# kcoost/fast_speech_enhancement_metrics

Measured on AMD Instinct MI355X. Metric: utterances/sec PESQ-wb+STOI, 10s@16kHz, batch 4096, 1/2/4/8 MI355X, higher is better.
Workload: dtype f32; 1 GPU; PESQ-wb + STOI/ESTOI of 10 s @ 16 kHz fp32 pairs through the drop-in call PESQ_STOI(16000, use_gpu=True)(c, n) (fused joint entry, one read of the inputs) -> list of dicts; batch_per_gpu=4096, global_batch=4096, length=160000, parallelism=dp1 (utterance shards, RCCL all-gather of scores)

## Files before the change

### fast_speech_enhancement_metrics_amd/csrc/fsem_stoi.h

```cpp
#pragma once
#include "fsem_fft.h"
#include "fsem_resample.h"
#include "fsem_vad.h"

namespace fsem {
namespace stoi {

constexpr int NB = 15;
constexpr int NSEG = 30;
constexpr int VF = 64;
#ifndef FSEM_TOB_TF
#define FSEM_TOB_TF 32
#endif
constexpr int TF = FSEM_TOB_TF;
constexpr float kClip = 1.0f + 5.62341325190349f;

struct Rows {
  const int32_t *lens;
  int64_t ncap;
  int orig, nw;
  __device__ __forceinline__ int64_t n(int64_t b) const {
    if (!lens) return ncap;
    const int64_t v = lens[b];
    return v < 0 ? 0 : (v > ncap ? ncap : v);
  }
  __device__ __forceinline__ int64_t l10(int64_t b) const { return (n(b) * nw + orig - 1) / orig; }
  __device__ __forceinline__ int nv(int64_t b) const {
    const int64_t L10 = l10(b);
    return L10 >= 256 ? (int)((L10 - 256) / 128 + 1) : 0;
  }
};

__device__ __forceinline__ uint32_t peak_exponents(float c0, float c1, float c2, float c3, float d0, float d1,
                                                   float d2, float d3) {
  typedef unsigned short us2 __attribute__((ext_vector_type(2)));
  auto mx4 = [](float a, float b, float c, float d) {
    return __float_as_uint(__builtin_fmaxf(__builtin_fmaxf(__builtin_fabsf(a), __builtin_fabsf(b)),
                                           __builtin_fmaxf(__builtin_fabsf(c), __builtin_fabsf(d))));
  };
  const uint32_t mc = mx4(c0, c1, c2, c3), md = mx4(d0, d1, d2, d3);
  uint32_t e = ((mc >> 7) & 0xffff0000u) | (md >> 23);
  auto pmax = [](uint32_t x, uint32_t y) {
    return __builtin_bit_cast(uint32_t, __builtin_elementwise_max(__builtin_bit_cast(us2, x), __builtin_bit_cast(us2, y)));
  };
  e = pmax(e, dpp_mov<0x121>(e));
  e = pmax(e, dpp_mov<0x122>(e));
  e = pmax(e, dpp_mov<0x124>(e));
  e = pmax(e, dpp_mov<0x128>(e));
  e = pmax(e, (uint32_t)__builtin_amdgcn_update_dpp(0, (int)e, 0x142, 0xA, 0xF, false));
  e = pmax(e, (uint32_t)__builtin_amdgcn_update_dpp(0, (int)e, 0x143, 0xC, 0xF, false));
  return __builtin_amdgcn_readlane(e, 63);
}

#ifndef FSEM_SEG_T
#define FSEM_SEG_T 256
#endif
constexpr int SEG_T = FSEM_SEG_T;

inline int seg_blocks(int64_t tmax) { return tmax > 29 ? (int)((tmax - 29 + SEG_T - 1) / SEG_T) : 1; }

struct Geometry {
  int64_t L10;
  int NV, nv_ld, tmax;
  int64_t v_ld;
  int64_t y_ld;
  bool direct;
  int mode;
};

inline int make_geometry(int64_t length, int32_t sr, Geometry *g, ResampleKernel *rk) {
  g->direct = (sr == 10000);
  if (g->direct) {
    g->L10 = length;
    rk->orig = rk->nw = 1;
    rk->taps = 1;
    rk->width = 0;
  } else {
    const int rc = make_resample_kernel(sr, 10000, rk);
    if (rc != FSEM_OK) return rc;
    g->L10 = (rk->nw * length + rk->orig - 1) / rk->orig;
  }
  g->NV = g->L10 >= 256 ? (int)((g->L10 - 256) / 128 + 1) : 0;
  g->nv_ld = (int)align_up((size_t)(g->NV > 0 ? g->NV : 1), 64);
  g->v_ld = vad_ld(g->L10);
  g->tmax = g->NV > 2 ? g->NV - 2 : 1;
  g->y_ld = (int64_t)align_up((size_t)g->L10, 64);
  g->mode = g->direct ? 1 : ((sr == 16000) ? 0 : 2);
  return FSEM_OK;
}

struct Ws {
  float2 *vad;
  int *idx, *kept;
  float *tob;
  double *part;
  float *y10;
};
inline Ws layout(Arena &a, int64_t B, const Geometry &g) {
  Ws w;
  w.vad = a.take<float2>((size_t)B * (size_t)g.v_ld);
  w.idx = a.take<int>((size_t)B * g.nv_ld);
  w.kept = a.take<int>((size_t)B);
  w.tob = a.take<float>((size_t)(2 * B) * NB * (size_t)g.tmax);
  w.part = a.take<double>(2 * (size_t)B * (size_t)seg_blocks(g.tmax));
  w.y10 = a.take<float>((size_t)(2 * B) * (size_t)g.y_ld);
  return w;
}

int run(const float *ref, const float *deg, int64_t B, int64_t length, int64_t ld, const int32_t *lengths,
        int32_t sr, float *stoi_out, float *estoi_out, int32_t *kept_out, float *tob_out, int64_t tob_ld, void *ws,
        size_t ws_size, hipStream_t st);

}
}
```

### fast_speech_enhancement_metrics_amd/csrc/stoi.hip

```cpp
#include <algorithm>

#include "fsem_internal.h"
#include "fsem_stoi.h"

namespace fsem {
namespace stoi {

struct Src {
  const float *x;
  int64_t n;
};

__device__ __forceinline__ float sample10(const Src &s, int64_t o, int64_t L10, bool direct,
                                          const ResampleKernel &rk) {
  if (o < 0 || o >= L10) return 0.f;
  return direct ? s.x[o] : resample_at(s.x, s.n, o, rk);
}

__device__ __forceinline__ void vad_chunk(const float *__restrict__ y, int n, float2 *__restrict__ vrow, int tid,
                                          float4 wa, float4 wb) {
  const int lane = tid & 63, grp = tid >> 4;
  const float4 *__restrict__ y4 = reinterpret_cast<const float4 *>(y);
  for (int j0 = 0; 64 * j0 < n; j0 += 16) {
    const int j = j0 + grp;
    const bool full = 64 * j + 64 <= n;
    const float4 v = full ? y4[16 * j + (lane & 15)] : make_float4(0.f, 0.f, 0.f, 0.f);
    const float e = vad_quarter(v, wa, wb, lane);
    if ((lane & 14) == 0 && full) reinterpret_cast<float *>(vrow)[2 * j + (lane & 1)] = e;
  }
}

constexpr int VF2 = 32;
constexpr int YT = VF2 * 128 + 128;
constexpr int NG = YT / 5 + 2;
constexpr int XT4 = (8 * NG + 32) / 4;
constexpr int XPF = (XT4 + 255) / 256;
__global__ void __launch_bounds__(256, 2)
    stoi_resample_vad16(const float *__restrict__ ref, const float *__restrict__ deg, Rows rows, int64_t ld,
                        int nchunk, int64_t nitems, float *__restrict__ y10, int64_t y_ld,
                        float2 *__restrict__ vad, int64_t v_ld) {
  __shared__ __attribute__((aligned(16))) float xin[XPF * 256 * 4 + 4];
  __shared__ __attribute__((aligned(16))) float ytile[YT + 8];
  const int tid = threadIdx.x, lane = tid & 63;
  const int wave = __builtin_amdgcn_readfirstlane(tid >> 6);
  auto item_src = [&](int64_t item, int64_t &b, int &chunk, int &sig, int64_t &o0, int64_t &i0) {
    sig = (int)(item & 1);
    const int64_t bc = item >> 1;
    b = bc / nchunk;
    chunk = (int)(bc - b * nchunk);
    o0 = (int64_t)chunk * (VF2 * 128);
    i0 = 8 * (o0 / 5) - 12;
  };
  auto prefetch = [&](int64_t item, float4 pre[XPF]) {
    int64_t b, o0, i0;
    int chunk, sig;
    item_src(item, b, chunk, sig, o0, i0);
    const int64_t n_in = rows.n(b);
    const uint32_t nbytes = (uint32_t)(((n_in + 3) & ~(int64_t)3) * 4);
    const float *row = (sig == 0 ? ref : deg) + b * ld;
    const uint64_t base = reinterpret_cast<uint64_t>(row);
    const uint32_t lo = __builtin_amdgcn_readfirstlane((uint32_t)base);
    const uint32_t hi = __builtin_amdgcn_readfirstlane((uint32_t)(base >> 32));
    void *p = reinterpret_cast<void *>(((uint64_t)hi << 32) | lo);
    const __amdgpu_buffer_rsrc_t rsrc =
        __builtin_amdgcn_make_buffer_rsrc(p, 0, __builtin_amdgcn_readfirstlane(nbytes), 0x00020000);
#pragma unroll
    for (int k = 0; k < XPF; ++k) {
      const int64_t t = i0 + 4 * (tid + 256 * k);
      typedef float v4f __attribute__((ext_vector_type(4)));
      v4f v = __builtin_bit_cast(v4f, __builtin_amdgcn_raw_buffer_load_b128(rsrc, (int)(t * 4), 0, 0));
      if (t + 3 >= n_in) {
        v.x = (t < n_in) ? v.x : 0.f;
        v.y = (t + 1 < n_in) ? v.y : 0.f;
        v.z = (t + 2 < n_in) ? v.z : 0.f;
        v.w = 0.f;
      }
      pre[k] = make_float4(v.x, v.y, v.z, v.w);
    }
  };
  float4 vwa, vwb;
  vad_windows(lane, (tid >> 4) & 1, vwa, vwb);
  float4 pre[XPF];
  int64_t item = blockIdx.x;
  if (item < nitems) prefetch(item, pre);
  for (; item < nitems; item += gridDim.x) {
    int64_t b, o0, i0;
    int chunk, sig;
    item_src(item, b, chunk, sig, o0, i0);
    const int64_t L10 = rows.l10(b);
    if (o0 >= L10) {
      if (item + gridDim.x < nitems) prefetch(item + gridDim.x, pre);
      continue;
    }
    float2 *x2 = reinterpret_cast<float2 *>(xin + 2);
#pragma unroll
    for (int k = 0; k < XPF; ++k) {
      x2[2 * (tid + 256 * k)] = make_float2(pre[k].x, pre[k].y);
      x2[2 * (tid + 256 * k) + 1] = make_float2(pre[k].z, pre[k].w);
    }
    lds_barrier();
    if (item + gridDim.x < nitems) prefetch(item + gridDim.x, pre);
    const int64_t o_end = min(o0 + (int64_t)YT, L10);
    const int64_t m0 = o0 / 5;
    const int64_t m1 = (o_end + 4) / 5;
    for (int64_t m = m0 + tid; m < m1; m += 256) {
      const float4 *xs4 = reinterpret_cast<const float4 *>(xin + 8 * (m - m0) + 4);
      float v[28];
#pragma unroll
      for (int t = 0; t < 7; ++t) {
        const float4 q = xs4[t];
        v[4 * t] = q.x;
        v[4 * t + 1] = q.y;
        v[4 * t + 2] = q.z;
        v[4 * t + 3] = q.w;
      }
#pragma unroll
      for (int j = 0; j < 5; ++j) {
        float acc = 0.f;
#pragma unroll
        for (int t = 0; t < 28; ++t) acc = fmaf(kRs16k10k[j][t], v[t], acc);
        const int64_t o = 5 * m + j;
        if (o >= o0 && o < o_end) ytile[o - o0] = acc;
      }
    }
    lds_barrier();
    const int nown = (int)min((int64_t)(VF2 * 128), L10 - o0);
    float *__restrict__ yr = y10 + (b * 2 + sig) * y_ld + o0;
    for (int k = tid; 4 * k < nown; k += 256) {
      if (4 * k + 3 < nown) {
        reinterpret_cast<float4 *>(yr)[k] = reinterpret_cast<const float4 *>(ytile)[k];
      } else {
        for (int c = 4 * k; c < nown; ++c) yr[c] = ytile[c];
      }
    }
    if (sig == 0) vad_chunk(ytile, nown, vad + b * v_ld + (o0 >> 6), tid, vwa, vwb);
    lds_barrier();
  }
}

constexpr int VF3 = 32;
constexpr int YT3 = VF3 * 128 + 128;
__global__ void __launch_bounds__(256)
    stoi_resample_vad(const float *__restrict__ ref, const float *__restrict__ deg, Rows rows, int64_t ld,
                      int mode, ResampleKernel rk, float *__restrict__ y10, int64_t y_ld,
                      float2 *__restrict__ vad, int64_t v_ld, int64_t b0) {
  __shared__ __attribute__((aligned(16))) float ytile[YT3];
  const int tid = threadIdx.x, lane = tid & 63;
  const int64_t b = b0 + blockIdx.y;
  const int64_t o0 = (int64_t)blockIdx.x * (VF3 * 128);
  const int64_t n_in = rows.n(b), L10 = rows.l10(b);
  if (o0 >= L10) return;
  const int64_t o_end = min(o0 + (int64_t)YT3, L10);
  const int ny = (int)(o_end - o0);
  const int nw_own = (int)min((int64_t)(VF3 * 128), L10 - o0);
  float4 vwa, vwb;
  vad_windows(lane, (tid >> 4) & 1, vwa, vwb);
  for (int sig = 0; sig < 2; ++sig) {
    const Src src{(sig == 0 ? ref : deg) + b * ld, n_in};
    for (int k = tid; k < ny; k += 256) ytile[k] = sample10(src, o0 + k, L10, mode == 1, rk);
    lds_barrier();
    float *__restrict__ yr = y10 + (b * 2 + sig) * y_ld + o0;
    for (int k = tid; k < nw_own; k += 256) yr[k] = ytile[k];
    if (sig == 0) vad_chunk(ytile, nw_own, vad + b * v_ld + (o0 >> 6), tid, vwa, vwb);
    lds_barrier();
  }
}

constexpr int VQ = 4096;
__global__ void __launch_bounds__(256)
    stoi_vad10(const float *__restrict__ y10, int64_t y_ld, Rows rows, float2 *__restrict__ vad, int64_t v_ld,
               int64_t b0) {
  const int64_t b = b0 + blockIdx.y;
  const int64_t o0 = (int64_t)blockIdx.x * VQ;
  const int64_t L10 = rows.l10(b);
  if (o0 >= L10) return;
  float4 vwa, vwb;
  vad_windows(threadIdx.x & 63, (threadIdx.x >> 4) & 1, vwa, vwb);
  vad_chunk(y10 + (2 * b) * y_ld + o0, (int)min((int64_t)VQ, L10 - o0), vad + b * v_ld + (o0 >> 6), threadIdx.x, vwa,
            vwb);
}

__global__ void __launch_bounds__(256)
    stoi_select(const float2 *__restrict__ vad, int64_t v_ld, int nv_ld, Rows rows, int *__restrict__ idx,
                int *__restrict__ kept) {
  __shared__ float red[8];
  __shared__ int wcount[4];
  const int tid = threadIdx.x, lane = tid & 63;
  const int wave = __builtin_amdgcn_readfirstlane(tid >> 6);
  const int64_t b = blockIdx.x;
  const int NV = rows.nv(b);
  const float2 *__restrict__ q = vad + b * v_ld;
  float m = -INFINITY;
  int nan_seen = 0;
  for (int i = tid; i < NV; i += 256) {
    const float e = vad_energy_db(q, i);
    m = fmaxf(m, e);
    nan_seen |= (e != e);
  }
  m = block_max_256(m, red);
  const float thr = __syncthreads_or(nan_seen) ? __builtin_nanf("") : m - 40.f;
  int base = 0;
  for (int i0 = 0; i0 < NV; i0 += 256) {
    const int i = i0 + tid;
    const bool keep = (i < NV) && ((thr - vad_energy_db(q, i)) < 0.f);
    const unsigned long long bal = __ballot(keep);
    const int pre = __popcll(bal & ((1ull << lane) - 1ull));
    if (lane == 0) wcount[wave] = __popcll(bal);
    lds_barrier();
    int off = base;
    for (int w = 0; w < wave; ++w) off += wcount[w];
    if (keep) idx[b * nv_ld + off + pre] = i;
    base += wcount[0] + wcount[1] + wcount[2] + wcount[3];
    lds_barrier();
  }
  if (tid == 0) kept[b] = base;
}

#ifdef FSEM_STAMPS
constexpr int kTobStampBlocks = 131072;
__device__ unsigned long long g_tob_stamps[kTobStampBlocks][4];
#define TSTAMP(i)                                                                            \
  do {                                                                                       \
    const unsigned lin_ = blockIdx.y * gridDim.x + blockIdx.x;                               \
    if (threadIdx.x == 0 && lin_ < kTobStampBlocks) g_tob_stamps[lin_][i] = __builtin_amdgcn_s_memtime(); \
  } while (0)
#else
#define TSTAMP(i) \
  do {            \
  } while (0)
#endif

constexpr int TOB_PB = 264;
__device__ __forceinline__ constexpr int tob_pw(int k) { return k + (k >= 128 ? 3 : 0); }
constexpr bool tob_pieces_unsplit() {
  for (int l = 0; l < 64; ++l)
    if (kObmPiece[l][2] < 128 && kObmPiece[l][3] > 128) return false;
  return true;
}
static_assert(tob_pieces_unsplit() && 2 * TOB_PB <= 2 * kFftBuf - 12, "padded band-sum layout");

constexpr int TOB_WAVES = 4;
__global__ void __launch_bounds__(64 * TOB_WAVES)
    stoi_tob(const float *__restrict__ y10, int64_t y_ld, int64_t B, Rows rows, const int *__restrict__ idx,
             const int *__restrict__ kept, int nv_ld, float *__restrict__ tob, int64_t tmax, int64_t b0) {
  __shared__ __attribute__((aligned(16))) float blk[2][TF + 1][128];
  __shared__ __attribute__((aligned(16))) float xbuf[TOB_WAVES * 2 * kFftBuf];
  const int tid = threadIdx.x, lane = tid & 63;
  const int wave = __builtin_amdgcn_readfirstlane(tid >> 6);
  const int64_t b = b0 + blockIdx.y;
  const int n = kept[b];
  const int T = n - 2;
  const int64_t L10 = rows.l10(b);
  const int k0 = blockIdx.x * TF;
  if (k0 >= T) return;
  TSTAMP(0);
  const int kend = min(k0 + TF, T);
  const int *kidx = idx + b * nv_ld;
  const float *__restrict__ yc = y10 + (b * 2) * y_ld;
  const float *__restrict__ yd = yc + y_ld;
  auto row_rsrc = [L10](const float *y) {
    const uint64_t base = reinterpret_cast<uint64_t>(y);
    const uint32_t lo = __builtin_amdgcn_readfirstlane((uint32_t)base);
    const uint32_t hi = __builtin_amdgcn_readfirstlane((uint32_t)(base >> 32));
    void *p = reinterpret_cast<void *>(((uint64_t)hi << 32) | lo);
    return __builtin_amdgcn_make_buffer_rsrc(p, 0, __builtin_amdgcn_readfirstlane((uint32_t)(L10 * 4)), 0x00020000);
  };
  const __amdgpu_buffer_rsrc_t rc = row_rsrc(yc), rd = row_rsrc(yd);
  auto at = [](__amdgpu_buffer_rsrc_t r, int64_t o) {
    return __builtin_bit_cast(float, __builtin_amdgcn_raw_buffer_load_b32(r, (int)(o * 4), 0, 0));
  };
  const float w_lo = kHann256s[lane], w_lo2 = kHann256s[lane + 64];
  const float w_hi = kHann256s[128 + lane], w_hi2 = kHann256s[128 + 64 + lane];

  const int nblk = kend - k0 + 1;
  constexpr int NBW = (TF + 1 + TOB_WAVES - 1) / TOB_WAVES;
  float g[NBW][8];
#pragma unroll
  for (int u = 0; u < NBW; ++u) {
    const int j = min(wave + TOB_WAVES * u, nblk - 1);
    const int q = k0 + 1 + j;
    const int iq = kidx[q], ip = kidx[q - 1];
    const int64_t a0 = 128LL * iq, a1 = 128LL * ip + 128;
    g[u][0] = at(rc, a0 + lane);
    g[u][1] = at(rc, a1 + lane);
    g[u][2] = at(rc, a0 + 64 + lane);
    g[u][3] = at(rc, a1 + 64 + lane);
    g[u][4] = at(rd, a0 + lane);
    g[u][5] = at(rd, a1 + lane);
    g[u][6] = at(rd, a0 + 64 + lane);
    g[u][7] = at(rd, a1 + 64 + lane);
  }
#pragma unroll
  for (int u = 0; u < NBW; ++u) {
    const int j = wave + TOB_WAVES * u;
    if (j < nblk) {
      blk[0][j][lane] = w_lo * g[u][0] + w_hi * g[u][1];
      blk[0][j][64 + lane] = w_lo2 * g[u][2] + w_hi2 * g[u][3];
      blk[1][j][lane] = w_lo * g[u][4] + w_hi * g[u][5];
      blk[1][j][64 + lane] = w_lo2 * g[u][6] + w_hi2 * g[u][7];
    }
  }
  lds_stores_done();
  lds_barrier();
  TSTAMP(1);

  cf tw1[8], tw2[8];
  fft512_twiddles(lane, tw1, tw2);
  const float win[4] = {w_lo, w_lo2, w_hi, w_hi2};
  float2 *wbuf = reinterpret_cast<float2 *>(xbuf) + wave * kFftBuf;
  float *pbuf = reinterpret_cast<float *>(wbuf);
  const int plane = (64 - lane) & 63;
  const int pc_sig = kObmPiece[lane][0], pc_band = kObmPiece[lane][1];
  const int pc_lo = kObmPiece[lane][2], pc_hi = kObmPiece[lane][3];
  const int pc_at = TOB_PB * pc_sig + tob_pw(pc_lo);
  const int pc_gs = kObmPiece[lane][4];
  const bool pc_head = kObmPiece[lane][5] != 0;
  const int nfr = kend - k0;
  const int nfft = 2 * ((nfr + 1) >> 1);
  for (int f = wave; f < nfft; f += TOB_WAVES) {
    const int sg = f & 1;
    const int ja = 2 * (f >> 1);
    const bool has_b = ja + 1 < nfr;
    cf v[8];
#pragma unroll
    for (int r = 0; r < 4; ++r) {
      const int t = lane + 64 * (r & 1);
      const float a = blk[sg][ja + (r >> 1)][t];
      const float bq = has_b ? blk[sg][ja + 1 + (r >> 1)][t] : 0.f;
      v[r] = {a * win[r], bq * win[r]};
    }
#pragma unroll
    for (int r = 4; r < 8; ++r) v[r] = {0.f, 0.f};
    const uint32_t pk = peak_exponents(v[0].r, v[1].r, v[2].r, v[3].r, v[0].i, v[1].i, v[2].i, v[3].i);
    const int ea = (int)(pk >> 16), eb = (int)(pk & 0xffffu);
    const bool a_zero = ea == 0 && !__any(v[0].r != 0.f || v[1].r != 0.f || v[2].r != 0.f || v[3].r != 0.f);
    const bool b_zero = eb == 0 && !__any(v[0].i != 0.f || v[1].i != 0.f || v[2].i != 0.f || v[3].i != 0.f);
    int sh = (ea > 0 && eb > 0) ? ea - eb : 0;
    sh = (sh >= 7 || sh <= -7) ? max(-60, min(60, sh)) : 0;
    if (sh != 0) {
#pragma unroll
      for (int r = 0; r < 4; ++r) v[r].i = __builtin_amdgcn_ldexpf(v[r].i, sh);
    }
    const float a_scale = a_zero ? 0.f : 0.5f;
    const float b_scale = b_zero ? 0.f : __builtin_amdgcn_ldexpf(0.5f, -sh);
    fft512_wave<true>(v, wbuf, lane, tw1, tw2);
    float pa[4], pb[4];
#pragma unroll
    for (int r = 0; r < 4; ++r) {
      float mr = __shfl(v[7 - r].r, plane, 64);
      float mi = __shfl(v[7 - r].i, plane, 64);
      if (lane == 0) {
        mr = v[(8 - r) & 7].r;
        mi = v[(8 - r) & 7].i;
      }
      typedef float f2v __attribute__((ext_vector_type(2)));
      const f2v z = {v[r].r, v[r].i}, m = {mr, mi};
      const f2v sm = z + m;
      const f2v df = z.yx - m.yx;
      const f2v pp = __builtin_elementwise_fma(sm, sm, df * df);
      pa[r] = pp.x;
      pb[r] = pp.y;
    }
#pragma unroll
    for (int r = 0; r < 4; ++r) {
      pbuf[tob_pw(64 * r) + lane] = pa[r];
      pbuf[TOB_PB + tob_pw(64 * r) + lane] = pb[r];
    }
    wave_lds_fence();
    {
      const float *ps = pbuf + pc_at;
      float acc = (pc_lo < pc_hi) ? ps[0] : 0.f;
#pragma unroll
      for (int i = 1; i < 12; ++i) {
        const float x = ps[i];
        acc += (pc_lo + i < pc_hi) ? x : 0.f;
      }
      {
        const float a1 = __builtin_bit_cast(float, __builtin_amdgcn_update_dpp(0, __builtin_bit_cast(int, acc), 0x101, 0xF, 0xF, true));
        acc += (pc_gs >= 2) ? a1 : 0.f;
        const float a2 = __builtin_bit_cast(float, __builtin_amdgcn_update_dpp(0, __builtin_bit_cast(int, acc), 0x102, 0xF, 0xF, true));
        acc += (pc_gs >= 4) ? a2 : 0.f;
      }
      if (pc_head && (pc_sig == 0 || has_b))
        tob[((b + sg * B) * NB + pc_band) * tmax + k0 + ja + pc_sig] =
            __builtin_amdgcn_sqrtf(acc) * (pc_sig ? b_scale : a_scale);
    }
    wave_lds_fence();
  }
  TSTAMP(2);
}

#ifndef FSEM_SEG_OCC
#define FSEM_SEG_OCC 3
#endif
constexpr int SEG_WAVES = SEG_T / 64;
typedef float f2 __attribute__((ext_vector_type(2)));
__global__ void __launch_bounds__(SEG_T, FSEM_SEG_OCC)
    stoi_seg(const float *__restrict__ tob, int64_t B, int64_t tmax, const int *__restrict__ kept,
             double *__restrict__ part, int P, int64_t b0) {
  constexpr int W = SEG_T + NSEG;
  constexpr int LDX = W + 1;
  __shared__ f2 XY[NB][LDX];
  __shared__ double red[2 * SEG_WAVES];
  const int tid = threadIdx.x;
  const int64_t b = b0 + blockIdx.y;
  const int p = blockIdx.x;
  const int n = kept[b];
  const int S = n - 31;
  const int m0 = p * SEG_T;
  if (m0 >= S) return;
  const int T = n - 2;
  const float *xc = tob + (b * NB) * tmax;
  const float *xd = tob + ((b + B) * NB) * tmax;
  double st = 0.0, et = 0.0;
  constexpr float kInvN = 1.f / NSEG;
  {
    const int nf = min(W, T - m0);
    {
      f2 va[NB], vb[NB];
      const int t2 = tid + SEG_T;
      const int ia = min(tid, nf - 1), ib = min(t2, nf - 1);
#pragma unroll
      for (int j = 0; j < NB; ++j) {
        const float *xr = xc + j * tmax + m0, *dr = xd + j * tmax + m0;
        va[j] = (f2){xr[ia], dr[ia]};
        vb[j] = (f2){xr[ib], dr[ib]};
      }
#pragma unroll
      for (int j = 0; j < NB; ++j) {
        XY[j][tid] = va[j];
        if (t2 < W) XY[j][t2] = vb[j];
      }
    }
    lds_barrier();
    const int m = m0 + tid;
    if (m < S) {
      float s_acc = 0.f;
      f2 rxy[NB], nmr[NB];
      f2 nvar = {0.f, 0.f};
#pragma unroll 1
      for (int j = 0; j < NB; ++j) {
        f2 v[NSEG];
        f2 s1 = {0.f, 0.f};
#pragma unroll
        for (int t = 0; t < NSEG; ++t) {
          v[t] = XY[j][tid + t];
          s1 += v[t];
        }
        const f2 mu = s1 * kInvN;
        f2 dd = {0.f, 0.f};
#pragma unroll
        for (int t = 0; t < NSEG; ++t) {
          v[t] = v[t] - mu;
          dd = __builtin_elementwise_fma(v[t], v[t], dd);
        }
        const f2 s2 = __builtin_elementwise_fma(mu * (float)NSEG, mu, dd);
        const float alpha = __builtin_amdgcn_sqrtf(s2.x) * __builtin_amdgcn_rcpf(__builtin_amdgcn_sqrtf(s2.y) + 1e-9f);
        const f2 sc = {kClip, alpha};
        const f2 smu = sc * mu;
        static_assert(NSEG % 2 == 0, "frame pairs");
        f2 c[NSEG / 2];
        f2 syc2 = {0.f, 0.f};
#pragma unroll
        for (int u = 0; u < NSEG / 2; ++u) {
          const f2 q0 = __builtin_elementwise_fma(v[2 * u], sc, smu), q1 = __builtin_elementwise_fma(v[2 * u + 1], sc, smu);
          c[u] = (f2){fminf(q0.y, q0.x), fminf(q1.y, q1.x)};
          syc2 += c[u];
        }
        const float myc = (syc2.x + syc2.y) * kInvN;
        const f2 myc2 = {myc, myc};
        f2 dcc2 = {0.f, 0.f};
        float dxc = 0.f;
#pragma unroll
        for (int u = 0; u < NSEG / 2; ++u) {
          const f2 dc = c[u] - myc2;
          dcc2 = __builtin_elementwise_fma(dc, dc, dcc2);
          dxc = fmaf(v[2 * u].x, dc.x, dxc);
          dxc = fmaf(v[2 * u + 1].x, dc.y, dxc);
        }
        const float dcc = dcc2.x + dcc2.y;
        constexpr float kReg30 = 30e-24f;
        const float rxn = __builtin_amdgcn_rsqf(dd.x + kReg30);
        const float ryn = __builtin_amdgcn_rsqf(dd.y + kReg30);
        const float rcn = __builtin_amdgcn_rsqf(dcc + kReg30);
        s_acc = fmaf(dxc * rxn, rcn, s_acc) + (__builtin_isfinite(alpha) ? 0.f : __builtin_nanf(""));
        rxy[j] = (f2){rxn, ryn};
        nvar = __builtin_elementwise_fma(rxy[j], rxy[j], nvar);
        nmr[j] = -mu * rxy[j];
      }
      const f2 breg = __builtin_elementwise_fma(nvar, (f2){14e-24f / 15.f, 14e-24f / 15.f}, (f2){15e-24f, 15e-24f});
      float e_acc = 0.f;
      for (int t = 0; t < NSEG; ++t) {
        f2 a[NB];
        f2 ma = {0.f, 0.f};
#pragma unroll
        for (int j = 0; j < NB; ++j) {
          a[j] = __builtin_elementwise_fma(XY[j][tid + t], rxy[j], nmr[j]);
          ma += a[j];
        }
        ma *= 1.f / NB;
        f2 q = {0.f, 0.f};
        float ac = 0.f;
#pragma unroll
        for (int j = 0; j < NB; ++j) {
          const f2 d = a[j] - ma;
          q = __builtin_elementwise_fma(d, d, q);
          ac = fmaf(d.x, d.y, ac);
        }
        const float ra = __builtin_amdgcn_rsqf(q.x + breg.x);
        const float rc = __builtin_amdgcn_rsqf(q.y + breg.y);
        e_acc = fmaf(ac * ra, rc, e_acc);
      }
      st += (double)s_acc;
      et += (double)e_acc;
    }
  }
  st = wave_sum_d(st);
  et = wave_sum_d(et);
  lds_barrier();
  if ((tid & 63) == 0) {
    red[(tid >> 6) * 2] = st;
    red[(tid >> 6) * 2 + 1] = et;
  }
  lds_barrier();
  if (tid == 0) {
    double a = red[0], e = red[1];
#pragma unroll
    for (int w = 1; w < SEG_WAVES; ++w) {
      a += red[2 * w];
      e += red[2 * w + 1];
    }
    part[(b * P + p) * 2] = a;
    part[(b * P + p) * 2 + 1] = e;
  }
}

__global__ void __launch_bounds__(256)
    stoi_seg_sum(const double *__restrict__ part, int P, int64_t B, const int *__restrict__ kept,
                 float *__restrict__ stoi_out, float *__restrict__ estoi_out) {
  const int64_t b = blockIdx.x * (int64_t)blockDim.x + threadIdx.x;
  if (b >= B) return;
  const int S = kept[b] - 31;
  if (S <= 0) {
    stoi_out[b] = __builtin_nanf("");
    estoi_out[b] = __builtin_nanf("");
    return;
  }
  const int np = (S + SEG_T - 1) / SEG_T;
  const double *q = part + b * P * 2;
  double st = 0.0, et = 0.0;
  for (int p = 0; p < np; ++p) {
    st += q[2 * p];
    et += q[2 * p + 1];
  }
  stoi_out[b] = (float)(st / NB / S);
  estoi_out[b] = (float)(et / NSEG / S);
}

inline int run_seg(int64_t B, const float *tob, int64_t tmax, const int *kept, double *part, float *stoi_out,
                   float *estoi_out, hipStream_t st) {
  const int P = seg_blocks(tmax);
  for (int64_t b0 = 0; b0 < B; b0 += kMaxGridY) {
    hipLaunchKernelGGL(stoi_seg, grid_slice((unsigned)P, B, b0), dim3(SEG_T), 0, st, tob, B, tmax, kept, part, P,
                       b0);
    FSEM_CHECK_LAUNCH();
  }
  hipLaunchKernelGGL(stoi_seg_sum, dim3((unsigned)((B + 255) / 256)), dim3(256), 0, st, part, P, B, kept, stoi_out,
                     estoi_out);
  FSEM_CHECK_LAUNCH();
  return FSEM_OK;
}

inline int run_tail(int64_t B, const Geometry &g, const Rows &rows, const float *y10, const float2 *vad, int *idx,
                    int *kept, float *tob, int64_t tmax, double *part, float *stoi_out, float *estoi_out,
                    hipStream_t st) {
  hipLaunchKernelGGL(stoi_select, dim3((unsigned)B), dim3(256), 0, st, vad, g.v_ld, g.nv_ld, rows, idx, kept);
  FSEM_CHECK_LAUNCH();
  for (int64_t b0 = 0; b0 < B; b0 += kMaxGridY) {
    hipLaunchKernelGGL(stoi_tob, grid_slice((unsigned)((g.tmax + TF - 1) / TF), B, b0), dim3(64 * TOB_WAVES), 0, st,
                       y10, g.y_ld, B, rows, idx, kept, g.nv_ld, tob, tmax, b0);
    FSEM_CHECK_LAUNCH();
  }
  if (stoi_out) return run_seg(B, tob, tmax, kept, part, stoi_out, estoi_out, st);
  return FSEM_OK;
}

int run(const float *ref, const float *deg, int64_t B, int64_t length, int64_t ld,
        const int32_t *lengths, int32_t sr, float *stoi_out, float *estoi_out, int32_t *kept_out,
        float *tob_out, int64_t tob_ld, void *ws, size_t ws_size, hipStream_t st) {
  Geometry g;
  ResampleKernel rk;
  int rc = make_geometry(length, sr, &g, &rk);
  if (rc != FSEM_OK) return rc;
  if (g.NV <= 0 && !lengths) return FSEM_ESHORT;
  const Rows rows{lengths, length, rk.orig, rk.nw};
  Arena a(ws);
  Ws w = layout(a, B, g);
  if (!a.fits(ws_size)) return FSEM_EWORKSPACE;
  int64_t tmax = g.tmax;
  if (tob_out) {
    w.tob = tob_out;
    tmax = tob_ld;
  }
  if (kept_out) w.kept = kept_out;
  if (g.mode == 0) {
    const int nchunk = (int)((g.L10 + VF2 * 128 - 1) / (VF2 * 128));
    const int64_t nitems = B * (int64_t)nchunk * 2;
    const int ncu = cu_count();
    const int64_t grid = nitems < (int64_t)ncu * 3 ? nitems : (int64_t)ncu * 3;
    hipLaunchKernelGGL(stoi_resample_vad16, dim3((unsigned)grid), dim3(256), 0, st, ref, deg, rows, ld, nchunk,
                       nitems, w.y10, g.y_ld, w.vad, g.v_ld);
  } else if (g.mode == 2) {
    rc = launch_resample_tiled(ref, B, length, ld, lengths, w.y10, 2 * g.y_ld, 0, rk, st);
    if (rc != FSEM_OK) return rc;
    rc = launch_resample_tiled(deg, B, length, ld, lengths, w.y10 + g.y_ld, 2 * g.y_ld, 0, rk, st);
    if (rc != FSEM_OK) return rc;
    for (int64_t b0 = 0; b0 < B; b0 += kMaxGridY) {
      hipLaunchKernelGGL(stoi_vad10, grid_slice((unsigned)((g.L10 + VQ - 1) / VQ), B, b0), dim3(256), 0, st, w.y10,
                         g.y_ld, rows, w.vad, g.v_ld, b0);
      FSEM_CHECK_LAUNCH();
    }
  } else {
    for (int64_t b0 = 0; b0 < B; b0 += kMaxGridY) {
      hipLaunchKernelGGL(stoi_resample_vad, grid_slice((unsigned)((g.L10 + VF3 * 128 - 1) / (VF3 * 128)), B, b0),
                         dim3(256), 0, st, ref, deg, rows, ld, g.mode, rk, w.y10, g.y_ld, w.vad, g.v_ld, b0);
      FSEM_CHECK_LAUNCH();
    }
  }
  FSEM_CHECK_LAUNCH();
  return run_tail(B, g, rows, w.y10, w.vad, w.idx, w.kept, w.tob, tmax, w.part, stoi_out, estoi_out, st);
}

}
}

using namespace fsem;

extern "C" size_t fsem_stoi_workspace_bytes(int64_t batch, int64_t length, int32_t sample_rate) {
  stoi::Geometry g;
  ResampleKernel rk;
  if (stoi::make_geometry(length, sample_rate, &g, &rk) != FSEM_OK) return 0;
  return layout_bytes(stoi::layout, batch, g);
}

extern "C" int fsem_stoi_f32(const float *ref, const float *deg, int64_t batch, int64_t length, int64_t ld,
                             const int32_t *lengths, int32_t sample_rate, float *stoi_out, float *estoi_out,
                             void *ws, size_t ws_bytes, void *stream) {
  if (!ref || !deg || !stoi_out || !estoi_out || batch <= 0 || length <= 0 || ld < length || length > kMaxLength)
    return FSEM_EINVAL;
  return stoi::run(ref, deg, batch, length, ld, lengths, sample_rate, stoi_out, estoi_out, nullptr, nullptr, 0,
                   ws, ws_bytes, (hipStream_t)stream);
}

extern "C" int fsem_stoi_tob_f32(const float *ref10, const float *deg10, int64_t batch, int64_t length10,
                                 int64_t ld, int32_t *kept, float *tob, int64_t tmax, void *ws, size_t ws_bytes,
                                 void *stream) {
  if (!ref10 || !deg10 || !kept || !tob || batch <= 0 || length10 <= 0 || ld < length10 || length10 > kMaxLength)
    return FSEM_EINVAL;
  stoi::Geometry g;
  ResampleKernel rk;
  int rc = stoi::make_geometry(length10, 10000, &g, &rk);
  if (rc != FSEM_OK) return rc;
  if (tmax < g.tmax) return FSEM_EINVAL;
  return stoi::run(ref10, deg10, batch, length10, ld, nullptr, 10000, nullptr, nullptr, kept, tob, tmax, ws,
                   ws_bytes, (hipStream_t)stream);
}

struct JointWs {
  pesq::WbWs pesq;
  stoi::Ws stoi;
};
static JointWs joint_layout(Arena &a, int64_t batch, int64_t length, const stoi::Geometry &g) {
  JointWs w;
  w.pesq = pesq::wb_layout(a, batch, length);
  w.stoi = stoi::layout(a, batch, g);
  return w;
}

extern "C" size_t fsem_pesq_stoi_workspace_bytes(int64_t batch, int64_t length) {
  stoi::Geometry g;
  ResampleKernel rk;
  if (stoi::make_geometry(length, 16000, &g, &rk) != FSEM_OK) return 0;
  return layout_bytes(joint_layout, batch, length, g);
}

extern "C" int fsem_pesq_stoi_f32(const float *ref, const float *deg, int64_t batch, int64_t length, int64_t ld,
                                  const int32_t *lengths, float *mos, float *stoi_out, float *estoi_out, void *ws,
                                  size_t ws_bytes, void *stream) {
  if (!ref || !deg || !mos || !stoi_out || !estoi_out || batch <= 0 || length <= 0 || ld < length ||
      length > kMaxLength)
    return FSEM_EINVAL;
  stoi::Geometry g;
  ResampleKernel rk;
  int rc = stoi::make_geometry(length, 16000, &g, &rk);
  if (rc != FSEM_OK) return rc;
  if (!lengths && (g.NV <= 0 || fsem_pesq_frames(length) < 20)) return FSEM_ESHORT;
  Arena a(ws);
  const JointWs jw = joint_layout(a, batch, length, g);
  if (!a.fits(ws_bytes)) return FSEM_EWORKSPACE;
  const pesq::WbWs &p = jw.pesq;
  const stoi::Ws &w = jw.stoi;
  const stoi::Rows rows{lengths, length, rk.orig, rk.nw};
  hipStream_t st = (hipStream_t)stream;
  const hipStream_t side = side_stream(st);
  const bool early = pesq::back_waves(batch, length) > 1;
  rc = pesq::launch_front(ref, deg, batch, length, ld, lengths, p.bark, p.power, p.front, w.y10, g.y_ld, w.vad,
                          g.v_ld, st, false);
  if (rc != FSEM_OK) return rc;
  if (early) {
    rc = stream_wait(side, st);
    if (rc != FSEM_OK) return rc;
    rc = pesq::launch_back(p.bark, nullptr, &p.front, batch, length, lengths, mos, p.back, side);
    if (rc != FSEM_OK) return rc;
    rc = stoi::run_tail(batch, g, rows, w.y10, w.vad, w.idx, w.kept, w.tob, g.tmax, w.part, stoi_out, estoi_out,
                        st);
  } else {
    rc = stoi::run_tail(batch, g, rows, w.y10, w.vad, w.idx, w.kept, w.tob, g.tmax, w.part, nullptr, nullptr, st);
    if (rc != FSEM_OK) return rc;
    rc = stream_wait(side, st);
    if (rc != FSEM_OK) return rc;
    rc = pesq::launch_back(p.bark, nullptr, &p.front, batch, length, lengths, mos, p.back, side);
    if (rc != FSEM_OK) return rc;
    rc = stoi::run_seg(batch, w.tob, g.tmax, w.kept, w.part, stoi_out, estoi_out, st);
  }
  const int rj = stream_wait(st, side);
  return rc != FSEM_OK ? rc : rj;
}

#ifdef FSEM_STAMPS
extern "C" int fsem_debug_read_tob_stamps(void *dst, size_t bytes) {
  if (hipDeviceSynchronize() != hipSuccess) return FSEM_ELAUNCH;
  return hipMemcpyFromSymbol(dst, HIP_SYMBOL(stoi::g_tob_stamps), bytes, 0, hipMemcpyDeviceToHost) == hipSuccess
             ? FSEM_OK : FSEM_ELAUNCH;
}
#endif
```

Before: 584,800 utterances/s.

## Split STOI third-octave kernel into single-wave per-signal blocks with smaller frame tiles

Restructures stoi_tob so each workgroup is a single wave that handles one signal (clean or degraded) over 10 frames instead of four waves handling both signals over 32 frames. This shrinks the LDS footprint per workgroup and multiplies the grid size, with occupancy set via launch bounds. The peak-exponent reduction is replaced with a permlane32_swap-based magnitude max that also removes the __any zero checks. Loads are batched ahead of use, both in the shuffles and in the band sums. The trade-off is that the window/index loads are repeated per signal and per smaller tile.

```diff
diff --git a/fast_speech_enhancement_metrics_amd/csrc/fsem_stoi.h b/fast_speech_enhancement_metrics_amd/csrc/fsem_stoi.h
--- a/fast_speech_enhancement_metrics_amd/csrc/fsem_stoi.h
+++ b/fast_speech_enhancement_metrics_amd/csrc/fsem_stoi.h
@@ -9,10 +9,7 @@
 constexpr int NB = 15;
 constexpr int NSEG = 30;
 constexpr int VF = 64;
-#ifndef FSEM_TOB_TF
-#define FSEM_TOB_TF 32
-#endif
-constexpr int TF = FSEM_TOB_TF;
+constexpr int TF = 32;
 constexpr float kClip = 1.0f + 5.62341325190349f;
 
 struct Rows {
@@ -50,6 +47,26 @@
   e = pmax(e, (uint32_t)__builtin_amdgcn_update_dpp(0, (int)e, 0x142, 0xA, 0xF, false));
   e = pmax(e, (uint32_t)__builtin_amdgcn_update_dpp(0, (int)e, 0x143, 0xC, 0xF, false));
   return __builtin_amdgcn_readlane(e, 63);
+}
+
+struct Peaks {
+  uint32_t a, b;
+};
+__device__ __forceinline__ Peaks peak_magnitudes(float c0, float c1, float c2, float c3, float d0, float d1, float d2,
+                                                 float d3) {
+  auto mx4 = [](float a, float b, float c, float d) {
+    return __float_as_uint(__builtin_fmaxf(__builtin_fmaxf(__builtin_fabsf(a), __builtin_fabsf(b)),
+                                           __builtin_fmaxf(__builtin_fabsf(c), __builtin_fabsf(d))));
+  };
+  const auto sw = __builtin_amdgcn_permlane32_swap(mx4(c0, c1, c2, c3), mx4(d0, d1, d2, d3), false, false);
+  uint32_t e = max(sw[0], sw[1]);
+  auto step = [](uint32_t x, uint32_t moved) { return max(x, moved); };
+  e = step(e, (uint32_t)__builtin_amdgcn_update_dpp(0, (int)e, 0x121, 0xF, 0xF, false));
+  e = step(e, (uint32_t)__builtin_amdgcn_update_dpp(0, (int)e, 0x122, 0xF, 0xF, false));
+  e = step(e, (uint32_t)__builtin_amdgcn_update_dpp(0, (int)e, 0x124, 0xF, 0xF, false));
+  e = step(e, (uint32_t)__builtin_amdgcn_update_dpp(0, (int)e, 0x128, 0xF, 0xF, false));
+  e = step(e, (uint32_t)__builtin_amdgcn_update_dpp(0, (int)e, 0x142, 0xA, 0xF, false));
+  return {(uint32_t)__builtin_amdgcn_readlane(e, 31), (uint32_t)__builtin_amdgcn_readlane(e, 63)};
 }
 
 #ifndef FSEM_SEG_T
diff --git a/fast_speech_enhancement_metrics_amd/csrc/stoi.hip b/fast_speech_enhancement_metrics_amd/csrc/stoi.hip
--- a/fast_speech_enhancement_metrics_amd/csrc/stoi.hip
+++ b/fast_speech_enhancement_metrics_amd/csrc/stoi.hip
@@ -239,11 +239,30 @@
 }
 static_assert(tob_pieces_unsplit() && 2 * TOB_PB <= 2 * kFftBuf - 12, "padded band-sum layout");
 
-constexpr int TOB_WAVES = 4;
-__global__ void __launch_bounds__(64 * TOB_WAVES)
+#ifndef FSEM_TOB_WAVES
+#define FSEM_TOB_WAVES 1
+#endif
+#ifndef FSEM_TOB_TF
+#define FSEM_TOB_TF 10
+#endif
+#ifndef FSEM_TOB_SPLIT
+#define FSEM_TOB_SPLIT 1
+#endif
+constexpr int TOB_WAVES = FSEM_TOB_WAVES;
+constexpr int TOB_TF = FSEM_TOB_TF;
+constexpr bool TOB_SPLIT = FSEM_TOB_SPLIT != 0;
+constexpr int TOB_NSIG = TOB_SPLIT ? 1 : 2;
+constexpr int TOB_LDS = (TOB_NSIG * (TOB_TF + 1) * 128 + TOB_WAVES * 2 * kFftBuf) * (int)sizeof(float);
+constexpr int TOB_FIT = 160 * 1024 / TOB_LDS * TOB_WAVES / 4;
+constexpr int TOB_OCC = TOB_FIT < 4 ? TOB_FIT : 4;
+static_assert(TOB_TF % 2 == 0, "frame pairs");
+static_assert(TOB_OCC >= 1, "stoi_tob: LDS per workgroup");
+inline unsigned tob_grid_x(int64_t tmax) { return (unsigned)((tmax + TOB_TF - 1) / TOB_TF) * (TOB_SPLIT ? 2u : 1u); }
+
+__global__ void __launch_bounds__(64 * TOB_WAVES, TOB_OCC)
     stoi_tob(const float *__restrict__ y10, int64_t y_ld, int64_t B, Rows rows, const int *__restrict__ idx,
              const int *__restrict__ kept, int nv_ld, float *__restrict__ tob, int64_t tmax, int64_t b0) {
-  __shared__ __attribute__((aligned(16))) float blk[2][TF + 1][128];
+  __shared__ __attribute__((aligned(16))) float blk[TOB_NSIG][TOB_TF + 1][128];
   __shared__ __attribute__((aligned(16))) float xbuf[TOB_WAVES * 2 * kFftBuf];
   const int tid = threadIdx.x, lane = tid & 63;
   const int wave = __builtin_amdgcn_readfirstlane(tid >> 6);
@@ -251,13 +270,12 @@
   const int n = kept[b];
   const int T = n - 2;
   const int64_t L10 = rows.l10(b);
-  const int k0 = blockIdx.x * TF;
+  const int wsig = TOB_SPLIT ? (int)(blockIdx.x & 1) : 0;
+  const int k0 = (int)(TOB_SPLIT ? blockIdx.x >> 1 : blockIdx.x) * TOB_TF;
   if (k0 >= T) return;
   TSTAMP(0);
-  const int kend = min(k0 + TF, T);
+  const int kend = min(k0 + TOB_TF, T);
   const int *kidx = idx + b * nv_ld;
-  const float *__restrict__ yc = y10 + (b * 2) * y_ld;
-  const float *__restrict__ yd = yc + y_ld;
   auto row_rsrc = [L10](const float *y) {
     const uint64_t base = reinterpret_cast<uint64_t>(y);
     const uint32_t lo = __builtin_amdgcn_readfirstlane((uint32_t)base);
@@ -265,7 +283,7 @@
     void *p = reinterpret_cast<void *>(((uint64_t)hi << 32) | lo);
     return __builtin_amdgcn_make_buffer_rsrc(p, 0, __builtin_amdgcn_readfirstlane((uint32_t)(L10 * 4)), 0x00020000);
   };
-  const __amdgpu_buffer_rsrc_t rc = row_rsrc(yc), rd = row_rsrc(yd);
+  const __amdgpu_buffer_rsrc_t rs[2] = {row_rsrc(y10 + (b * 2 + wsig) * y_ld), row_rsrc(y10 + (b * 2 + 1) * y_ld)};
   auto at = [](__amdgpu_buffer_rsrc_t r, int64_t o) {
     return __builtin_bit_cast(float, __builtin_amdgcn_raw_buffer_load_b32(r, (int)(o * 4), 0, 0));
   };
@@ -273,31 +291,31 @@
   const float w_hi = kHann256s[128 + lane], w_hi2 = kHann256s[128 + 64 + lane];
 
   const int nblk = kend - k0 + 1;
-  constexpr int NBW = (TF + 1 + TOB_WAVES - 1) / TOB_WAVES;
-  float g[NBW][8];
+  constexpr int NBW = (TOB_TF + 1 + TOB_WAVES - 1) / TOB_WAVES;
+  float g[NBW][TOB_NSIG][4];
 #pragma unroll
   for (int u = 0; u < NBW; ++u) {
     const int j = min(wave + TOB_WAVES * u, nblk - 1);
     const int q = k0 + 1 + j;
     const int iq = kidx[q], ip = kidx[q - 1];
     const int64_t a0 = 128LL * iq, a1 = 128LL * ip + 128;
-    g[u][0] = at(rc, a0 + lane);
-    g[u][1] = at(rc, a1 + lane);
-    g[u][2] = at(rc, a0 + 64 + lane);
-    g[u][3] = at(rc, a1 + 64 + lane);
-    g[u][4] = at(rd, a0 + lane);
-    g[u][5] = at(rd, a1 + lane);
-    g[u][6] = at(rd, a0 + 64 + lane);
-    g[u][7] = at(rd, a1 + 64 + lane);
+#pragma unroll
+    for (int s = 0; s < TOB_NSIG; ++s) {
+      g[u][s][0] = at(rs[s], a0 + lane);
+      g[u][s][1] = at(rs[s], a1 + lane);
+      g[u][s][2] = at(rs[s], a0 + 64 + lane);
+      g[u][s][3] = at(rs[s], a1 + 64 + lane);
+    }
   }
 #pragma unroll
   for (int u = 0; u < NBW; ++u) {
     const int j = wave + TOB_WAVES * u;
     if (j < nblk) {
-      blk[0][j][lane] = w_lo * g[u][0] + w_hi * g[u][1];
-      blk[0][j][64 + lane] = w_lo2 * g[u][2] + w_hi2 * g[u][3];
-      blk[1][j][lane] = w_lo * g[u][4] + w_hi * g[u][5];
-      blk[1][j][64 + lane] = w_lo2 * g[u][6] + w_hi2 * g[u][7];
+#pragma unroll
+      for (int s = 0; s < TOB_NSIG; ++s) {
+        blk[s][j][lane] = w_lo * g[u][s][0] + w_hi * g[u][s][1];
+        blk[s][j][64 + lane] = w_lo2 * g[u][s][2] + w_hi2 * g[u][s][3];
+      }
     }
   }
   lds_stores_done();
@@ -316,25 +334,29 @@
   const int pc_gs = kObmPiece[lane][4];
   const bool pc_head = kObmPiece[lane][5] != 0;
   const int nfr = kend - k0;
-  const int nfft = 2 * ((nfr + 1) >> 1);
+  const int nfft = TOB_NSIG * ((nfr + 1) >> 1);
   for (int f = wave; f < nfft; f += TOB_WAVES) {
-    const int sg = f & 1;
-    const int ja = 2 * (f >> 1);
+    const int ls = TOB_SPLIT ? 0 : f & 1;
+    const int sg = TOB_SPLIT ? wsig : ls;
+    const int ja = TOB_SPLIT ? 2 * f : 2 * (f >> 1);
     const bool has_b = ja + 1 < nfr;
+    const uint32_t b_mask = has_b ? 0xffffffffu : 0u;
     cf v[8];
+    float xa[4], xb[4];
 #pragma unroll
     for (int r = 0; r < 4; ++r) {
       const int t = lane + 64 * (r & 1);
-      const float a = blk[sg][ja + (r >> 1)][t];
-      const float bq = has_b ? blk[sg][ja + 1 + (r >> 1)][t] : 0.f;
-      v[r] = {a * win[r], bq * win[r]};
-    }
+      xa[r] = blk[ls][ja + (r >> 1)][t];
+      xb[r] = blk[ls][ja + 1 + (r >> 1)][t];
+    }
+#pragma unroll
+    for (int r = 0; r < 4; ++r)
+      v[r] = {xa[r] * win[r], __uint_as_float(__float_as_uint(xb[r] * win[r]) & b_mask)};
 #pragma unroll
     for (int r = 4; r < 8; ++r) v[r] = {0.f, 0.f};
-    const uint32_t pk = peak_exponents(v[0].r, v[1].r, v[2].r, v[3].r, v[0].i, v[1].i, v[2].i, v[3].i);
-    const int ea = (int)(pk >> 16), eb = (int)(pk & 0xffffu);
-    const bool a_zero = ea == 0 && !__any(v[0].r != 0.f || v[1].r != 0.f || v[2].r != 0.f || v[3].r != 0.f);
-    const bool b_zero = eb == 0 && !__any(v[0].i != 0.f || v[1].i != 0.f || v[2].i != 0.f || v[3].i != 0.f);
+    const Peaks pk = peak_magnitudes(v[0].r, v[1].r, v[2].r, v[3].r, v[0].i, v[1].i, v[2].i, v[3].i);
+    const int ea = (int)(pk.a >> 23), eb = (int)(pk.b >> 23);
+    const bool a_zero = pk.a == 0, b_zero = pk.b == 0;
     int sh = (ea > 0 && eb > 0) ? ea - eb : 0;
     sh = (sh >= 7 || sh <= -7) ? max(-60, min(60, sh)) : 0;
     if (sh != 0) {
@@ -344,11 +366,15 @@
     const float a_scale = a_zero ? 0.f : 0.5f;
     const float b_scale = b_zero ? 0.f : __builtin_amdgcn_ldexpf(0.5f, -sh);
     fft512_wave<true>(v, wbuf, lane, tw1, tw2);
-    float pa[4], pb[4];
+    float pa[4], pb[4], sr[4], si[4];
 #pragma unroll
     for (int r = 0; r < 4; ++r) {
-      float mr = __shfl(v[7 - r].r, plane, 64);
-      float mi = __shfl(v[7 - r].i, plane, 64);
+      sr[r] = __shfl(v[7 - r].r, plane, 64);
+      si[r] = __shfl(v[7 - r].i, plane, 64);
+    }
+#pragma unroll
+    for (int r = 0; r < 4; ++r) {
+      float mr = sr[r], mi = si[r];
       if (lane == 0) {
         mr = v[(8 - r) & 7].r;
         mi = v[(8 - r) & 7].i;
@@ -369,12 +395,12 @@
     wave_lds_fence();
     {
       const float *ps = pbuf + pc_at;
-      float acc = (pc_lo < pc_hi) ? ps[0] : 0.f;
-#pragma unroll
-      for (int i = 1; i < 12; ++i) {
-        const float x = ps[i];
-        acc += (pc_lo + i < pc_hi) ? x : 0.f;
-      }
+      float x[12];
+#pragma unroll
+      for (int i = 0; i < 12; ++i) x[i] = ps[i];
+      float acc = (pc_lo < pc_hi) ? x[0] : 0.f;
+#pragma unroll
+      for (int i = 1; i < 12; ++i) acc += (pc_lo + i < pc_hi) ? x[i] : 0.f;
       {
         const float a1 = __builtin_bit_cast(float, __builtin_amdgcn_update_dpp(0, __builtin_bit_cast(int, acc), 0x101, 0xF, 0xF, true));
         acc += (pc_gs >= 2) ? a1 : 0.f;
@@ -577,7 +603,7 @@
   hipLaunchKernelGGL(stoi_select, dim3((unsigned)B), dim3(256), 0, st, vad, g.v_ld, g.nv_ld, rows, idx, kept);
   FSEM_CHECK_LAUNCH();
   for (int64_t b0 = 0; b0 < B; b0 += kMaxGridY) {
-    hipLaunchKernelGGL(stoi_tob, grid_slice((unsigned)((g.tmax + TF - 1) / TF), B, b0), dim3(64 * TOB_WAVES), 0, st,
+    hipLaunchKernelGGL(stoi_tob, grid_slice(tob_grid_x(g.tmax), B, b0), dim3(64 * TOB_WAVES), 0, st,
                        y10, g.y_ld, B, rows, idx, kept, g.nv_ld, tob, tmax, b0);
     FSEM_CHECK_LAUNCH();
   }
```

After: 588,200 utterances/s (median of 5 runs). No clear change (+0.6%).
